# jonas089/toyni

Hardware: AMD Instinct MI355X
Metric: BabyBear NTT throughput (forward+inverse, device-resident) (higher is better)
Workload: dtype u32; 1 GPU; forward+inverse NTT n=2^20 (configs[1]) over a batch of 1024 transforms per GPU (configs[3] repeated-prover batch), in place, inputs resident in HBM; log_n=20, batch_per_gpu=1024, batch_total=1024, passes_per_transform=2, parallelism=batch-sharded x1, no collective

## Files before the change

toyni_amd/csrc/ntt_kernels.hpp:

```cpp
#pragma once
#include "bb_field.hpp"

namespace toyni {

enum PassKind : int { KIND_COL = 0, KIND_ROW_T = 1, KIND_ROW_N = 2 };

struct PassArgs {
    const uint32_t* in;
    uint32_t* out;
    const uint32_t* stage_tw;
    const uint32_t* stage_tw3;
    const uint32_t* tw_lo;
    const uint32_t* tw_hi;
    uint32_t tw_lowbits;
    uint32_t log_S;
    uint32_t scale;
    uint32_t log_n;
    uint32_t log_M1;
    uint32_t log_mid;
    uint64_t rows_total;
    const uint32_t* cs_lo;
    const uint32_t* cs_hi;
    uint32_t cs_lowbits;
    uint32_t cs_mode;
    uint32_t cs_g;
    uint32_t col_base;
    uint32_t in_prefix_log;
    uint32_t nz_rows;
    uint32_t in_split_shift, in_split_extra;
    uint32_t out_split_shift, out_split_extra, out_prefix_log;
    uint32_t row0;
    uint32_t seeds_invariant;
};

#ifndef TOYNI_ABLATE
#define TOYNI_ABLATE 0
#endif

template <bool NT = false>
TOYNI_HD uint32_t ld32(const uint32_t* base, uint32_t byte_off) {
#if TOYNI_ABLATE & 1
    return (uint32_t)(reinterpret_cast<uintptr_t>(base) >> 2) + byte_off;
#elif defined(__HIP_DEVICE_COMPILE__)
    if constexpr (NT) return __builtin_nontemporal_load(reinterpret_cast<const uint32_t*>(reinterpret_cast<const char*>(base) + byte_off));
    else return *reinterpret_cast<const uint32_t*>(reinterpret_cast<const char*>(base) + byte_off);
#else
    return *reinterpret_cast<const uint32_t*>(reinterpret_cast<const char*>(base) + byte_off);
#endif
}
template <bool NT = false>
TOYNI_HD void st32(uint32_t* base, uint32_t byte_off, uint32_t v) {
#if TOYNI_ABLATE & 2
    if (v == 0xFFFFFFFFu)
#endif
#if defined(__HIP_DEVICE_COMPILE__)
// ... 47 lines not shown
    static_assert(LQ_ == 0 || LQ_ == 2, "interleave: none, or the four coordinates of an Ext element");
    static_assert(LQ_ == 0 || KIND == KIND_COL || LC - LQ_ >= (KIND == KIND_ROW_T ? 2 : 3) || LE2 == 0, "interleaved rows: 4 or >= 8 rows per coordinate");
    static constexpr int LM = LE1 + LE2;
    static constexpr int LE1_ = LE1;
    static constexpr int STEPS = LE2 > 0 ? 2 : 1;
    static constexpr int IN_STEP_LOG = LE2, OUT_STEP_LOG = LE2 > 0 ? LE1 : 0;
    static constexpr bool NT = NT_;
    static constexpr uint32_t M = 1u << LM, E1 = 1u << LE1, E2 = 1u << LE2, C = 1u << LC;
    static constexpr uint32_t T = C * E2;
    static constexpr uint32_t G2 = E1 / E2;
    static constexpr bool TWO_STEP = LE2 > 0;

    static constexpr uint32_t PADC = C < 32 ? 32 - C : 0;
    static constexpr uint32_t HI_STRIDE = KIND == KIND_COL ? E2 * C + PADC : E2 + 1;
    static constexpr uint32_t LOW_STRIDE = KIND == KIND_COL ? C : 1;
    static constexpr uint32_t row_pitch() {
        uint32_t base = E1 * (E2 + 1);
        uint32_t want = KIND == KIND_ROW_T ? (C <= 16 ? 2u : 1u) : (LQ_ > 0 ? 1u : (E1 < 32 ? E1 : 0u));
        return base + ((want + 32u - (base & 31u)) & 31u);
    }
    static constexpr uint32_t PITCH = row_pitch();
    static constexpr uint32_t C_STRIDE = KIND == KIND_COL ? 1 : PITCH;
    static constexpr uint32_t LDS_WORDS = !TWO_STEP ? 0 : (KIND == KIND_COL ? E1 * HI_STRIDE : C * PITCH);

    static constexpr uint32_t lds_wg_per_cu() {
        return LDS_WORDS ? (160u * 1024u) / ((LDS_WORDS + (TWO_STEP ? M - E2 : 0u) + ((TWO_STEP && LE1 >= 2 && LC >= 4) ? M - 2u * E2 : 0u)) * 4u) : 8u;
    }
    static constexpr uint32_t min_waves_per_simd() {
        uint32_t w = (lds_wg_per_cu() * (T / 64u ? T / 64u : 1u) + 3u) / 4u;
        return w < 1u ? 1u : (w > 4u ? 4u : w);
    }
    static constexpr uint32_t MIN_WAVES = min_waves_per_simd();

    static TOYNI_HD uint32_t lds_row(uint32_t c) {
        if (LQ_ == 0 || KIND == KIND_COL) return c;
        const uint32_t q = c & (Q - 1u), cc = c >> LQ_;
        if ((C >> LQ_) >= 8u) return (q << 3) + (cc & 7u) + ((cc >> 3) << 5);
        return q * (C >> LQ_) + cc;
    }
    static TOYNI_HD uint32_t lds_word(uint32_t c, uint32_t hi, uint32_t low) { return lds_row(c) * C_STRIDE + hi * HI_STRIDE + low * LOW_STRIDE; }

    struct Tile {
        const uint32_t* in;
        uint32_t* out;
        uint32_t row_shift;
        uint32_t col0;
        uint32_t out0;
        uint32_t valid_c;
        uint32_t bidx;
// ... 100 lines not shown
        return r;
    }
    static TOYNI_HD Twiddle group_twiddle_finish(const PassArgs& a, const TwiddleRaw& r) {
        Twiddle tw{0u, 0u};
        if (KIND == KIND_COL) {
            tw.a0 = mont_mul(r.a_hi, r.a_lo);
            if (a.scale) tw.a0 = mont_mul(tw.a0, a.scale);
            tw.g = mont_mul(r.g_hi, r.g_lo);
        } else if (a.cs_mode == 2u) {
            tw.a0 = mont_mul(r.a_hi, r.a_lo);
            if (KIND == KIND_ROW_N && a.scale) tw.a0 = mont_mul(tw.a0, a.scale);
            tw.g = a.cs_g;
        } else if (SLAB_ && KIND == KIND_ROW_T && a.cs_mode == 4u) {
            tw.a0 = mont_mul(r.a_hi, r.a_lo);
            tw.g = mont_mul(r.g_hi, r.g_lo);
        }
        return tw;
    }
    template <int LSH>
    static TOYNI_HD Twiddle group_twiddle(const PassArgs& a, const Tile& t, uint32_t c, uint32_t khi) {
        return group_twiddle_finish(a, group_twiddle_issue<LSH>(a, t, c, khi));
    }

    template <int LB, int LSH>
    static TOYNI_HD void finish(const PassArgs& a, const Tile& t, uint32_t c, uint32_t khi, Twiddle twd, uint32_t (&x)[1 << LB]) {
        constexpr uint32_t NB = 1u << LB;
        const uint32_t off0 = out_offset(a, c, khi) << 2;
        const uint32_t step = (out_offset(a, 0u, 1u << LSH) - out_offset(a, 0u, 0u)) << 2;
        char* base = reinterpret_cast<char*>(t.out);
#if TOYNI_BUF
        const BufRsrc ws = buf_rsrc(base);
#define TOYNI_STORE(B, V) do { if constexpr (KIND != KIND_ROW_N) stb32<NT_>(ws, off0, (B) * step, (V)); \
                               else st32<NT_>(reinterpret_cast<uint32_t*>(base + (uint64_t)(B) * step), off0, (V)); } while (0)
#else
#define TOYNI_STORE(B, V) st32<NT_>(reinterpret_cast<uint32_t*>(base + (uint64_t)(B) * step), off0, (V))
#endif
        if (KIND == KIND_COL) {
            uint32_t tw = twd.a0;
#pragma unroll
            for (uint32_t b = 0; b < NB; ++b) {
                TOYNI_STORE(b, mont_mul(x[cx_bitrev(b, LB)], tw));
                if (b + 1 < NB) { tw = mont_mul_lazy(tw, twd.g); TOYNI_PIN(tw); }
            }
        } else if (SLAB_ && KIND == KIND_ROW_T) {
            uint32_t tw = twd.a0;
#pragma unroll
            for (uint32_t b = 0; b < NB; ++b) {
                const uint32_t piece = ((b << LSH) >> a.out_split_shift) * (a.out_split_extra << 2);
                uint32_t v = x[cx_bitrev(b, LB)];
                if (a.cs_mode == 4u) {
                    v = mont_mul(v, tw);
                    if (b + 1 < NB) { tw = mont_mul_lazy(tw, twd.g); TOYNI_PIN(tw); }
                }
#if TOYNI_BUF
                stb32<NT_>(ws, off0, b * step + piece, v);
#else
                st32<NT_>(reinterpret_cast<uint32_t*>(base + (uint64_t)b * step + piece), off0, v);
#endif
            }
        } else if (a.cs_mode == 2u) {
// ... 80 lines not shown
                if (q == 0) {
                    x[i + DP] = bb_sub(s0, s1);
                    const uint32_t t = mont_dot_sub(b, e, uni_pow<LE>(uni, QUARTER, false), uni_pow<LE>(uni, QUARTER, true));
                    x[i + D] = bb_add(d0, t);
                    x[i + D + DP] = bb_sub(d0, t);
                } else {
                    const uint32_t d1 = bb_sub(b, e);
                    x[i + DP] = mont_dot_sub(s0, s1, uni_pow<LE>(uni, 2u * q * G, false), uni_pow<LE>(uni, 2u * q * G, true));
                    x[i + D] = mont_dot2(d0, uni_pow<LE>(uni, q * G, false), d1, uni_pow<LE>(uni, q * G + QUARTER, false));
                    x[i + D + DP] = mont_dot2(d0, uni_pow<LE>(uni, 3u * q * G, false), d1, uni_pow<LE>(uni, 3u * q * G + QUARTER, true));
                }
            }
            stages_uniform_r4<LE, S - 2>(x, uni);
        } else if constexpr (S == 0) {
#pragma unroll
            for (uint32_t i = 0; i < (1u << LE); i += 2) {
                const uint32_t u = x[i], v = x[i + 1];
                x[i] = bb_add(u, v);
                x[i + 1] = bb_sub(u, v);
            }
        }
    }

    template <int LE, int SHIFT, int S>
    static TOYNI_HD void stages_thread_r4(uint32_t (&x)[1 << LE], const uint32_t* tw1, const uint32_t* tw3, uint32_t low) {
        TOYNI_PIN(low);
        if constexpr (S >= 1) {
            constexpr int t = S + SHIFT;
            constexpr uint32_t D = 1u << S, DP = 1u << (S - 1), HALF = 1u << (t - 1);
            const uint32_t* t1 = tw1 + ((1u << t) - (1u << SHIFT));
            const uint32_t* t2 = tw1 + (HALF - (1u << SHIFT));
            const uint32_t* t3 = tw3 + ((1u << t) - (2u << SHIFT));
            uint32_t n1 = t1[low], n1p = t1[low + HALF], n2 = t2[low], n3 = t3[low], n3n = t3[HALF + low];
#pragma unroll
            for (uint32_t q = 0; q < DP; ++q) {
                const uint32_t w1 = n1, w1p = n1p, w2 = n2, nw2 = BB_P - n2, w3 = n3, w3n = n3n;
                if (q + 1 < DP) {
                    const uint32_t e1 = low + ((q + 1) << SHIFT);
                    n1 = t1[e1]; n1p = t1[e1 + HALF]; n2 = t2[e1]; n3 = t3[e1]; n3n = t3[HALF + e1];
                }
                TOYNI_SCHED_FENCE();
#pragma unroll
                for (uint32_t hi = 0; hi < (1u << (LE - 1 - S)); ++hi) {
                    const uint32_t i = (hi << (S + 1)) | q;
                    const uint32_t a = x[i], b = x[i + DP], c = x[i + D], e = x[i + D + DP];
                    const uint32_t s0 = bb_add(a, c), s1 = bb_add(b, e), d0 = bb_sub(a, c), d1 = bb_sub(b, e);
                    x[i] = bb_add(s0, s1);
                    x[i + DP] = mont_dot_sub(s0, s1, w2, nw2);
                    x[i + D] = mont_dot2(d0, w1, d1, w1p);
                    x[i + D + DP] = mont_dot2(d0, w3, d1, w3n);
                }
            }
            stages_thread_r4<LE, SHIFT, S - 2>(x, tw1, tw3, low);
        } else if constexpr (S == 0) {
            const uint32_t w = tw1[low], nw = BB_P - w;
#pragma unroll
            for (uint32_t i = 0; i < (1u << LE); i += 2) {
                const uint32_t u = x[i], v = x[i + 1];
                x[i] = bb_add(u, v);
                x[i + 1] = mont_dot_sub(u, v, w, nw);
            }
        }
    }

    template <int LE, int SHIFT, bool R4T = false>
    static TOYNI_HD void stages(uint32_t (&x)[1 << LE], const uint32_t* tw1, uint32_t low, const uint32_t* uni, const uint32_t* tw3 = nullptr) {
#if !defined(TOYNI_NO_RADIX4)
        if constexpr (R4T && SHIFT > 0 && LE >= 2) {
            stages_thread_r4<LE, SHIFT, LE - 1>(x, tw1, tw3, low);
            return;
        }
        if constexpr (SHIFT == 0 && LE >= 2) {
            stages_uniform_r4<LE, LE - 1>(x, uni);
            return;
        }
#endif
#pragma unroll
        for (int s = LE - 1; s >= 0; --s) {
            const int d = 1 << s;
            const int t = s + SHIFT;
            uint32_t w[1 << (LE - 1)], nw[1 << (LE - 1)];
#pragma unroll
// ... 114 lines not shown
            r.lo = a.cs_lo[j0 & ((1u << a.cs_lowbits) - 1u)];
            r.hi = a.cs_hi[j0 >> a.cs_lowbits];
        }
        return r;
    }
    static TOYNI_HD uint32_t in_seed_finish(const PassArgs& a, const InSeedRaw& r) {
        return (KIND != KIND_ROW_T && a.cs_mode == 1u) ? mont_mul(r.hi, r.lo) : 0u;
    }
    template <int LZ = 0>
    static TOYNI_HD void in_scale(const PassArgs& a, const InSeedRaw& r, uint32_t (&x)[E1]) { in_scale_by<LZ>(a, in_seed_finish(a, r), x); }
    template <int LZ = 0>
    static TOYNI_HD void in_scale_by(const PassArgs& a, uint32_t seed, uint32_t (&x)[E1]) {
        constexpr uint32_t NZ = E1 >> (LZ < LE1 ? LZ : LE1);
        if (KIND != KIND_ROW_T && a.cs_mode == 1u) {
            uint32_t tw = seed;
#pragma unroll
            for (uint32_t i = 0; i < NZ; ++i) {
                x[i] = mont_mul(x[i], tw);
                if (i + 1 < NZ) { tw = mont_mul_lazy(tw, a.cs_g); TOYNI_PIN(tw); }
            }
        }
    }

    template <int LZ = 0>
    static TOYNI_HD void step1(const PassArgs& a, const Tile& t, uint32_t tid, uint32_t (&x)[E1], uint32_t* lds, const Uniform& uni,
                               const uint32_t* tw1, const uint32_t* tw3) {
        static_assert(LZ == 0 || TWO_STEP, "zero-padded input needs a two-step pass");
        uint32_t c, lo;
        coords1(tid, c, lo);
        if constexpr (LZ == 0) stages<LE1, LE2, STEP1_R4>(x, tw1, lo, uni.w, tw3);
        else stages_lz<LE1, LE2, LZ, LE1 - 1>(x, tw1, lo, uni.w);
        if (TWO_STEP) {
            const uint32_t base = lds_word(c, 0u, lo);
#pragma unroll
            for (uint32_t i = 0; i < E1; ++i) lds[base + i * HI_STRIDE] = x[i];
        } else {
            if (KIND != KIND_ROW_N || c < t.valid_c) finish<LE1, 0>(a, t, c, 0u, group_twiddle<0>(a, t, c, 0u), x);
        }
    }

    struct SeedsRaw { TwiddleRaw g[G2 ? G2 : 1]; };
    struct Seeds { Twiddle g[G2 ? G2 : 1]; };
    static TOYNI_HD SeedsRaw seeds_issue(const PassArgs& a, const Tile& t, uint32_t tid) {
        SeedsRaw s;
#pragma unroll
        for (uint32_t g = 0; g < G2; ++g) {
            uint32_t c, hi;
            coords2(tid, g, c, hi);
            s.g[g] = group_twiddle_issue<LE1>(a, t, c, bitrev32(hi, LE1));
        }
        return s;
    }
    static TOYNI_HD Seeds seeds_finish(const PassArgs& a, const SeedsRaw& r) {
        Seeds s;
#pragma unroll
        for (uint32_t g = 0; g < G2; ++g) s.g[g] = group_twiddle_finish(a, r.g[g]);
        return s;
    }

    static TOYNI_HD void step2(const PassArgs& a, const Tile& t, uint32_t tid, const uint32_t* lds, const Seeds& seeds, const Uniform& uni) {
#pragma unroll
        for (uint32_t g = 0; g < G2; ++g) {
            uint32_t c, hi;
            coords2(tid, g, c, hi);
            uint32_t x[E2];
            const uint32_t base = lds_word(c, hi, 0u);
#pragma unroll
            for (uint32_t i = 0; i < E2; ++i) x[i] = lds[base + i * LOW_STRIDE];
            stages<LE2, 0>(x, nullptr, 0u, uni.w);
            if (KIND != KIND_ROW_N || c < t.valid_c) finish<LE2, LE1>(a, t, c, bitrev32(hi, LE1), seeds.g[g], x);
        }
    }

    template <int LZ = 0>
    static TOYNI_HD void phase1(const PassArgs& a, uint32_t tile_id, uint32_t tid, uint32_t* lds) {
        const Tile t = tile_of(a, tile_id);
        uint32_t x[E1];
        load_tile<0, E1, LZ>(a, t, tid, x);
        in_scale<LZ>(a, in_seed_issue(a, t, tid), x);
        step1<LZ>(a, t, tid, x, lds, load_uniform(a), tw1_global(a), tw3_global(a));
    }
    static TOYNI_HD void phase2(const PassArgs& a, uint32_t tile_id, uint32_t tid, const uint32_t* lds) {
        const Tile t = tile_of(a, tile_id);
        step2(a, t, tid, lds, seeds_finish(a, seeds_issue(a, t, tid)), load_uniform(a));
    }
};

template <int KIND, int LE1, int LE2, int LE3, int LC, bool NT_ = false, int LQ_ = 0>
struct Pass3 {
    static_assert(KIND == KIND_COL || KIND == KIND_ROW_T, "passes of multi-pass plans");
    static_assert(LQ_ == 0 || (LQ_ == 2 && (LC == 2 || (LC == 4 && LE1 == 5))),
                  "interleaved tiles: one element's four coordinates (latency), or four rows / elements x four coordinates (streaming shapes)");
    static constexpr int LQ = LQ_;
    static_assert(LE1 >= LE2 && LE2 >= LE3 && LE3 >= 1 && LE1 <= 5, "step sizes");
    static constexpr int STEPS = 3;
    static constexpr bool STREAM = LE1 == 5;
    static constexpr int LM = LE1 + LE2 + LE3, LLO = LE2 + LE3, LHM = LE1 + LE2;
    static constexpr int IN_STEP_LOG = LLO, OUT_STEP_LOG = LHM;
    static constexpr bool NT = NT_;
    static constexpr uint32_t M = 1u << LM, E = 1u << LE1, E2 = 1u << LE2, E3 = 1u << LE3, C = 1u << LC;
    static constexpr uint32_t T = C << LLO;
    static constexpr uint32_t G2 = E / E2, G3 = E / E3;
    static_assert(T >= 64 && T <= 1024, "workgroup size");
    using Stg = Pass<KIND_ROW_N, 5, 5, 3>;

    static constexpr uint32_t PADC = C < 32 ? C : 0;
    static constexpr uint32_t PITCH = STREAM ? (M + (M >> LE3)) + ((2u + 32u - ((M + (M >> LE3)) & 31u)) & 31u) : ((M + (M >> LE3)) | 1u);
    static constexpr uint32_t LDS_WORDS = KIND == KIND_COL ? M * C + (M >> LE3) * PADC : C * PITCH;
    static constexpr uint32_t TW_WORDS = M - E3;
    static constexpr bool STEP1_R4 = STREAM;
    static constexpr uint32_t TW1S_WORDS = STREAM ? M - (1u << (LE2 + LE3)) : 0u;
    static constexpr uint32_t TW3S_WORDS = STEP1_R4 ? M - (2u << (LE2 + LE3)) : 0u;
    static constexpr uint32_t MIN_WAVES = 4;
    static constexpr uint32_t STRIDE1 = KIND == KIND_COL ? (C << LLO) + (PADC << LE2) : (1u << LLO) + (1u << LE2);
    static constexpr uint32_t STRIDE2 = KIND == KIND_COL ? (C << LE3) + PADC : E3 + 1u;
    static constexpr uint32_t STRIDE3 = KIND == KIND_COL ? C : 1u;
    static TOYNI_HD uint32_t lds_row(uint32_t c) {
        if (LQ_ == 0 || KIND == KIND_COL || C != 16u) return c;
// ... 742 lines not shown
```

toyni_amd/csrc/ntt_plan.hpp:

```cpp
#pragma once
#include <stdint.h>
#include <type_traits>
#include <vector>

#include "bb_field.hpp"
#include "ntt_kernels.hpp"
#include "ntt_route.hpp"

namespace toyni {

constexpr int MAX_PASSES = 3;
constexpr int MAX_LOG_N = 27;

struct PassPlan {
    int kind;
    int log_m;
    int log_s;
    uint32_t stage_off, stage3_off;
    uint32_t lo_off, hi_off, lowbits;
};

struct NttPlan {
    int log_n = 0;
    int npasses = 0;
// ... 285 lines not shown
    uint32_t log_parts = 0;
    const uint32_t* tw_lo = nullptr;
    const uint32_t* tw_hi = nullptr;
    uint32_t tw_lowbits = 0, row0 = 0;
    bool dry = false;
    bool* unsupported = nullptr;
};

template <class P> struct SlabVariant { using type = P; };
template <int K, int A, int B, int C, bool N, int Q> struct SlabVariant<Pass<K, A, B, C, N, Q, false>> { using type = Pass<K, A, B, C, false, Q, true>; };
template <class P> constexpr bool slab_variant_exists() {
    if constexpr (P::STEPS == 2) return P::PASS_KIND != KIND_ROW_N && P::LQ == 0 && P::C == 32u && P::LM >= 7 && P::LM <= 9 && !P::NT;
    else return false;
}

template <int LQ = 0, class Launch>
inline bool for_each_pass(const LaunchKnobs& k, const NttPlan& plan, const uint32_t* tables, bool inverse, const uint32_t* src,
                          uint32_t* work, uint32_t* dst, uint64_t batch, Launch&& launch, const CosetTables& cs = CosetTables(),
                          int lde_log = 0, bool nt = false, const SlabIo* sio = nullptr) {
    if (plan.log_n == 0 || batch == 0) return true;
    if (sio && (LQ != 0 || lde_log != 0 || cs.lo || plan.npasses < 2 || (batch & (batch - 1)) != 0 || (int)sio->log_parts >= plan.log_n)) return false;
    if (lde_log && (inverse || plan.npasses < 2 || lde_log > plan.pass[0].log_m)) return false;
    const uint64_t total_log = (uint64_t)plan.log_n;
    for (int p = 0; p < plan.npasses; ++p) {
        const PassPlan& pp = plan.pass[p];
        PassArgs a{};
        a.in = p == 0 ? src : work;
        a.out = p == plan.npasses - 1 ? dst : work;
        a.stage_tw = tables + pp.stage_off;
        a.stage_tw3 = tables + pp.stage3_off;
        a.tw_lo = tables + pp.lo_off;
        a.tw_hi = tables + pp.hi_off;
        a.tw_lowbits = pp.lowbits;
        a.log_S = (uint32_t)(pp.log_s + LQ);
        a.in_prefix_log = (uint32_t)(pp.log_s + pp.log_m - (p == 0 ? lde_log : 0) + LQ);
        a.nz_rows = (1u << pp.log_m) >> (p == 0 ? lde_log : 0);
        a.scale = (inverse && p == 0) ? plan.scale_inv : 0u;
        a.log_n = (uint32_t)plan.log_n;
        a.log_M1 = (uint32_t)plan.pass[0].log_m;
        a.log_mid = (uint32_t)(plan.log_n - plan.pass[0].log_m - pp.log_m);
        a.rows_total = batch;
        int log_tiles32 = 0;
        {
            const uint64_t tiles32 = (batch << (total_log - (uint64_t)pp.log_m)) >> 5;
            while ((2ull << log_tiles32) <= tiles32) ++log_tiles32;
        }
        auto body = [&](auto pass, auto lzc) {
            using P = decltype(pass);
            const bool cs_here = cs.lo && (inverse ? p == plan.npasses - 1 : p == 0);
            if (cs_here) {
                a.cs_lo = cs.lo;
                a.cs_hi = cs.hi;
                a.cs_lowbits = cs.lowbits;
                a.cs_mode = inverse ? 2u : 1u;
                uint64_t dj;
                if (!inverse) dj = pp.kind == KIND_COL ? (((uint64_t)1 << P::IN_STEP_LOG) << pp.log_s) : ((uint64_t)1 << P::IN_STEP_LOG);
                else dj = pp.kind == KIND_ROW_T ? ((uint64_t)1 << P::OUT_STEP_LOG) << (plan.log_n - P::LM)
                                                : ((uint64_t)1 << P::OUT_STEP_LOG);
                a.cs_g = to_mont_host(bb_pow_host(cs.s, dj));
            }
            uint64_t nblocks;
            if (pp.kind == KIND_ROW_N) nblocks = (batch + P::C - 1) / P::C;
            else nblocks = (batch << (total_log - P::LM)) / P::C;
            if (sio) {
                const uint32_t log_w = (uint32_t)plan.log_n - sio->log_parts;
                const uint32_t extra = (uint32_t)((batch - 1) << log_w);
                const bool first = p == 0, last = p == plan.npasses - 1;
                bool ok_shape = true;
                const bool special = (!inverse && first) || (inverse && last);
                if (!inverse && first) {
                    ok_shape = slab_variant_exists<P>() && pp.kind == KIND_COL && pp.log_m >= (int)sio->log_parts + P::IN_STEP_LOG;
// ... 6 lines not shown
                    a.out_prefix_log = log_w;
                    a.out_split_shift = (uint32_t)P::LM - sio->log_parts;
                    a.out_split_extra = extra;
                    a.cs_lo = sio->tw_lo;
                    a.cs_hi = sio->tw_hi;
                    a.cs_lowbits = sio->tw_lowbits;
                    a.cs_mode = 4u;
                    a.row0 = sio->row0;
                }
                if (batch == 1) ok_shape = false;
                if (!ok_shape) { if (sio->unsupported) *sio->unsupported = true; return; }
                if (sio->dry || (sio->unsupported && *sio->unsupported)) return;
                if constexpr (slab_variant_exists<P>() && decltype(lzc)::value == 0) {
                    if (special) { launch(typename SlabVariant<P>::type{}, lzc, a, nblocks); return; }
                }
            }
            launch(pass, lzc, a, nblocks);
        };
        bool ok;
        const bool slab_special = sio && ((!inverse && p == 0) || (inverse && p == plan.npasses - 1));
        if (slab_special && log_tiles32 >= k.wide_tiles) log_tiles32 = k.wide_tiles - 1;
        if (p == 0 && lde_log) ok = dispatch_pass_lz<LQ>(k, pp.log_m, log_tiles32, lde_log < 5 ? lde_log : 5, body);
        else ok = dispatch_pass<LQ>(k, pp.kind, pp.log_m, log_tiles32, [&](auto pass) { body(pass, std::integral_constant<int, 0>{}); }, nt && !slab_special);
        if (!ok) return false;
    }
    return true;
}

template <class Launch>
inline bool lds_transform(const NttPlan& plan, const uint32_t* tables, bool inverse, const uint32_t* src, uint32_t* dst, uint64_t batch,
                          Launch&& launch, const CosetTables& cs = CosetTables(), int log_rows = 5) {
    if (!plan.lds_la) return false;
    if (batch == 0) return true;
    LdsArgs g{};
    g.in = src;
    g.out = dst;
    g.stage_a = tables + plan.lds_stage_a_off;
    g.stage_b = tables + plan.lds_stage_b_off;
    g.gtab = tables + plan.lds_gtab_off;
    g.scale = inverse ? plan.scale_inv : 0u;
    g.batch = batch;
    if (cs.lo) {
        g.cs_lo = cs.lo;
        g.cs_hi = cs.hi;
        g.cs_lowbits = cs.lowbits;
        g.cs_mode = inverse ? 2u : 1u;
        g.cs_g = to_mont_host(bb_pow_host(cs.s, inverse ? (32ull << plan.lds_la) : 1024ull));
// ... 73 lines not shown
```

toyni_amd/csrc/ntt_route.hpp:

```cpp
#pragma once
#include <cstdlib>
#include <stdint.h>

namespace toyni {

inline int env_int(const char* name, int dflt) { const char* env = std::getenv(name); return env ? std::atoi(env) : dflt; }
inline uint64_t env_u64(const char* name, uint64_t dflt) { const char* env = std::getenv(name); return env ? (uint64_t)std::strtoull(env, nullptr, 0) : dflt; }

struct LaunchKnobs {
    int p3_tiles = 6;
    int lat_tiles = 7;
    int wide_tiles = 12;
    int s3_tiles = 7;
    bool split_small_first = true;
    int split3[3] = {0, 0, 0};
    int lds_max_log = 13;
    uint64_t lds_min_elems = (uint64_t)1 << 25;
    int lds_rows = 3;
    uint64_t r2048_min_rows = 2048;
    uint64_t r4096_min_rows = 2048;
    uint64_t nt_min_bytes = (uint64_t)512 << 20;

    static LaunchKnobs from_env() {
        LaunchKnobs k;
// ... 14 lines not shown
        if (const char* env = std::getenv("TOYNI_NO_LDS_KERNEL")) if (env[0] == '1') k.lds_max_log = 10;
        k.lds_min_elems = env_u64("TOYNI_LDS_MIN_ELEMS", k.lds_min_elems);
        k.lds_rows = env_int("TOYNI_LDS_ROWS", k.lds_rows);
        k.r2048_min_rows = env_u64("TOYNI_R2048_MIN_ROWS", k.r2048_min_rows);
        k.r4096_min_rows = env_u64("TOYNI_R4096_MIN_ROWS", k.r4096_min_rows);
        k.nt_min_bytes = env_u64("TOYNI_NT_MIN_BYTES", k.nt_min_bytes);
        return k;
    }
};

inline const LaunchKnobs& launch_knobs() {
    static const LaunchKnobs k = LaunchKnobs::from_env();
    return k;
}

constexpr bool seeds_launch_invariant(uint64_t grid, uint64_t ntiles, uint32_t log_S, uint32_t LC) {
    if (grid == 0 || log_S < LC) return false;
    if (grid >= ntiles) return true;
    const uint32_t tiles_log = log_S - LC;
    if (tiles_log == 0) return true;
    if (tiles_log >= 32) return false;
    if ((grid & (((uint64_t)1 << tiles_log) - 1)) != 0) return false;
    return (ntiles & 15) != 0 || (grid & 15) == 0;
}

inline bool has_latency_plan(int log_n) { return log_n == 21 || log_n == 22; }
inline bool has_stream2_plan(int log_n) { return log_n == 21; }

template <class Plan> inline bool row2048_enabled(const Plan& plan, uint64_t batch, const LaunchKnobs& k) {
    if (batch < 1) return false;
    return (plan.log_n == 11 && batch >= k.r2048_min_rows) || (plan.log_n == 12 && batch >= k.r4096_min_rows);
}
template <class Plan> inline bool lds_kernel_enabled(const Plan& plan, uint64_t batch, const LaunchKnobs& k) {
    return plan.lds_la != 0 && plan.log_n <= k.lds_max_log && (batch << plan.log_n) >= k.lds_min_elems;
}

template <class Plan> inline bool use_two_pass_plan(const Plan& plan, const Plan* plan_lat, uint64_t batch, int lq, int lde_log, const LaunchKnobs& k) {
    if (!plan_lat) return false;
    if (lde_log != 0 && lde_log > plan_lat->pass[0].log_m) return false;
    if (lq != 0) return (has_stream2_plan(plan.log_n) || (lde_log != 0 && has_latency_plan(plan.log_n))) && k.s3_tiles <= 7;
    const bool lat_small = k.p3_tiles >= 0 && k.lat_tiles >= 0 &&
                           ((batch << (plan.log_n - plan_lat->pass[0].log_m)) >> 5) <= (1ull << k.lat_tiles);
    const bool lat_stream = k.s3_tiles < 99 && (has_stream2_plan(plan.log_n) || (lde_log != 0 && has_latency_plan(plan.log_n)));
    return lat_small || lat_stream;
}

// ... 46 lines not shown
```

toyni_amd/csrc/toyni_hip.hip:

```cpp
#ifndef TOYNI_KERNEL_TEXT_ONLY
#include <hip/hip_runtime.h>

#include <cstdio>
#include <cstdlib>
#include <atomic>
#include <chrono>
#include <cstring>
#include <map>
#include <mutex>
#include <string>
#include <thread>
#include <vector>

#ifdef TOYNI_TOOLS
#include "toyni_hip_tools.h"
#endif
#endif
#include "toyni_hip.h"
#include "ntt_plan.hpp"
#include "merkle_kernels.hpp"
#include "prover_kernels.hpp"

using namespace toyni;

// ... 13 lines not shown
}
#undef hipLaunchKernelGGL
#define hipLaunchKernelGGL(kernel, grid, block, shmem, stream, ...)                                      \
    do {                                                                                                 \
        static std::atomic<bool> _toyni_site_seen{false};                                                \
        if (!_toyni_site_seen.load(std::memory_order_acquire)) {                                         \
            if (launch_registry::note(reinterpret_cast<const void*>(kernel)))                            \
                _toyni_site_seen.store(true, std::memory_order_release);                                 \
        }                                                                                                \
        kernel<<<(grid), (block), (shmem), (stream)>>>(__VA_ARGS__);                                     \
    } while (0)

#define HIPCHK(expr)                                 \
    do {                                               \
        hipError_t _e = (expr);                        \
        if (_e != hipSuccess) return (int)_e;          \
    } while (0)
#endif

template <class P> struct PassKindOf;
template <int K, int A, int B, int C, bool N, int Q, bool S> struct PassKindOf<Pass<K, A, B, C, N, Q, S>> { static constexpr int value = K; };
template <class P> constexpr int kind_of() { return PassKindOf<P>::value; }

template <class P, int PF, int LZ = 0>
__global__ void __launch_bounds__(P::T, P::MIN_WAVES) ntt_pass_kernel(const PassArgs a, const uint32_t ntiles) {
    __shared__ uint32_t lds[(P::LDS_WORDS + P::TW1_WORDS + P::TW3_WORDS) ? (P::LDS_WORDS + P::TW1_WORDS + P::TW3_WORDS) : 1];
    const uint32_t tid = threadIdx.x;
    if constexpr (!P::TWO_STEP) {
        static_assert(LZ == 0, "single-step passes take whole inputs");
        for (uint32_t v = blockIdx.x; v < ntiles; v += gridDim.x) P::phase1(a, P::tile_order(v, ntiles), tid, lds);
    } else {
        constexpr uint32_t NPF = PF < 0 ? 0u : ((uint32_t)PF > P::E1 ? P::E1 : (uint32_t)PF);
        uint32_t v = blockIdx.x;
        if (v >= ntiles) return;
        uint32_t* lds_tw1 = lds + P::LDS_WORDS;
        uint32_t* lds_tw3 = lds_tw1 + P::TW1_WORDS;
        uint32_t x[P::E1];
        typename P::Tile t = P::tile_of(a, P::tile_order(v, ntiles));
        P::template load_tile<0, NPF, LZ>(a, t, tid, x);
        typename P::SeedsRaw raw = P::seeds_issue(a, t, tid);
        typename P::InSeedRaw inraw = P::in_seed_issue(a, t, tid);
        const typename P::Uniform uni = P::load_uniform(a);
        for (uint32_t j = tid; j < P::TW1_WORDS; j += P::T) lds_tw1[j] = P::tw1_global(a)[j];
        for (uint32_t j = tid; j < P::TW3_WORDS; j += P::T) lds_tw3[j] = P::tw3_global(a)[j];
        TOYNI_WAIT_VMEM0();
        __syncthreads();
        const bool hoist = kind_of<P>() == KIND_COL && !P::SLAB && a.seeds_invariant != 0u;
        typename P::Seeds seeds = P::seeds_finish(a, raw);
        uint32_t inseed = P::in_seed_finish(a, inraw);
        while (true) {
            static_assert(P::G2 * P::E2 == P::E1 && P::E1 <= 63, "stores per tile per thread");
            if constexpr (kind_of<P>() != KIND_ROW_N) TOYNI_WAIT_VMEM_ALLOW(P::E1);
            else TOYNI_WAIT_VMEM0();
            P::template load_tile<NPF, P::E1, LZ>(a, t, tid, x);
            if (!hoist) inseed = P::in_seed_finish(a, inraw);
            P::template in_scale_by<LZ>(a, inseed, x);
            P::template step1<LZ>(a, t, tid, x, lds, uni, lds_tw1, lds_tw3);
            if (!hoist) seeds = P::seeds_finish(a, raw);
#pragma unroll
            for (uint32_t g = 0; g < P::G2; ++g) { TOYNI_PIN(seeds.g[g].a0); TOYNI_PIN(seeds.g[g].g); }
            TOYNI_SCHED_FENCE();
            const uint32_t vn = v + gridDim.x;
            const bool more = vn < ntiles;
            typename P::Tile tn = t;
            if (more) {
                tn = P::tile_of(a, P::tile_order(vn, ntiles));
                P::template load_tile<0, NPF, LZ>(a, tn, tid, x);
                if (!hoist) {
                    raw = P::seeds_issue(a, tn, tid);
                    inraw = P::in_seed_issue(a, tn, tid);
                }
            }
            TOYNI_SCHED_FENCE();
            TOYNI_LDS_BARRIER();
            TOYNI_SCHED_FENCE();
            P::step2(a, t, tid, lds, seeds, uni);
            if (!more) break;
            TOYNI_SCHED_FENCE();
            TOYNI_BARRIER();
            TOYNI_SCHED_FENCE();
            t = tn;
            v = vn;
        }
    }
}

template <class P, int LZ = 0>
__global__ void __launch_bounds__(P::T, P::MIN_WAVES) ntt_pass3_kernel(const PassArgs a, const uint32_t ntiles) {
    __shared__ uint32_t lds[P::LDS_WORDS + P::TW_WORDS];
    const uint32_t tid = threadIdx.x;
    uint32_t v = blockIdx.x;
    if (v >= ntiles) return;
    uint32_t* lds_tw = lds + P::LDS_WORDS;
    constexpr uint32_t TW_REGS = (P::TW_WORDS + P::T - 1) / P::T;
    uint32_t tw_regs[TW_REGS];
#pragma unroll
    for (uint32_t k = 0; k < TW_REGS; ++k) {
        const uint32_t j = tid + k * P::T;
        tw_regs[k] = j < P::TW_WORDS ? P::tw_global(a)[j] : 0u;
    }
    const typename P::Uniform uni = P::load_uniform(a);
    bool first = true;
    while (true) {
        const typename P::Tile t = P::tile_of(a, P::tile_order(v, ntiles));
        uint32_t x[P::E];
// ... 1485 lines not shown
    }
    (void)hipGetLastError();
    (void)hipThreadExchangeStreamCaptureMode(&cmode);
    for (size_t i = 0; i < c->retired.size(); ++i)
        if (!c->retired[i].ptr) drop_retired_event(c, i);
    size_t keep = 0;
    for (auto& r : c->retired)
        if (r.ptr) c->retired[keep++] = r;
    c->retired.resize(keep);
}

int grid_for(size_t items, int block = 256) {
    size_t g = (items + block - 1) / block;
    const size_t cap = 256 * 8;
    return (int)(g < 1 ? 1 : (g > cap ? cap : g));
}

template <class P> constexpr int ext_prefetch() { return (kind_of<P>() == KIND_ROW_N && P::LM == 10) ? 0 : 32; }

template <class P> constexpr bool hoists_seeds() {
    if constexpr (P::STEPS == 2) return kind_of<P>() == KIND_COL && !P::SLAB;
    else return false;
}

template <class P> constexpr uint32_t log_tile_width() {
    uint32_t l = 0;
    while ((1u << l) < P::C) ++l;
    return l;
}

template <class P, int LZ = 0>
void launch_pass(unsigned grid, hipStream_t s, const PassArgs& args, uint32_t ntiles) {
    PassArgs a = args;
    if constexpr (hoists_seeds<P>()) a.seeds_invariant = seeds_launch_invariant(grid, ntiles, a.log_S, log_tile_width<P>()) ? 1u : 0u;
    if constexpr (P::STEPS == 3) {
        if constexpr (P::STREAM) hipLaunchKernelGGL((ntt_pass3s_kernel<P, LZ>), dim3(grid), dim3(P::T), 0, s, a, ntiles);
        else hipLaunchKernelGGL((ntt_pass3_kernel<P, LZ>), dim3(grid), dim3(P::T), 0, s, a, ntiles);
    } else if constexpr (LZ > 0) {
        hipLaunchKernelGGL((ntt_pass_kernel<P, 32, LZ>), dim3(grid), dim3(P::T), 0, s, a, ntiles);
    } else if constexpr (P::LQ > 0) {
        hipLaunchKernelGGL((ntt_pass_kernel<P, ext_prefetch<P>()>), dim3(grid), dim3(P::T), 0, s, a, ntiles);
    } else {
        hipLaunchKernelGGL((ntt_pass_kernel<P, 32>), dim3(grid), dim3(P::T), 0, s, a, ntiles);
    }
}

template <class P, int LZ = 0>
unsigned persistent_grid(toyni_ntt_ctx* c, uint64_t ntiles) {
    static const int per_cu = [] {
        int occ = 0;
        hipError_t qe;
        if constexpr (P::STEPS == 3) {
            if constexpr (P::STREAM) qe = hipOccupancyMaxActiveBlocksPerMultiprocessor(&occ, ntt_pass3s_kernel<P, LZ>, (int)P::T, 0);
            else qe = hipOccupancyMaxActiveBlocksPerMultiprocessor(&occ, ntt_pass3_kernel<P, 0>, (int)P::T, 0);
        } else if constexpr (P::LQ > 0) qe = hipOccupancyMaxActiveBlocksPerMultiprocessor(&occ, ntt_pass_kernel<P, ext_prefetch<P>()>, (int)P::T, 0);
        else qe = hipOccupancyMaxActiveBlocksPerMultiprocessor(&occ, ntt_pass_kernel<P, 32>, (int)P::T, 0);
        if (qe != hipSuccess || occ < 1) occ = 1;
        if (const int v = env_int("TOYNI_WG_PER_CU", 0); v > 0) occ = v;
        return occ;
    }();
    uint64_t g = (uint64_t)c->num_cus * (uint64_t)per_cu;
    if (g > ntiles) g = ntiles;
    if (g >= 16) g &= ~(uint64_t)15;
    return (unsigned)(g < 1 ? 1 : g);
// ... 2061 lines not shown
```

Baseline: 306.7 billion elements/s.

## Fold inter-pass twiddle multiply into the closing row pass for 2^20 NTT

For the two-pass 1024x1024 plan, the column pass now stores plain outputs without the per-element twiddle multiply. The twiddles are instead folded into the first radix-4 stage of the row pass, which uses a per-tile LDS table of G factors. The final radix-2 stage then applies the A factor together with the inverse scale. This removes a separate multiply chain in the column pass. In exchange it adds an LDS table, per-tile twiddle loads, and mont_dot2 butterflies in the row pass, which may reduce occupancy.

```diff
diff --git a/toyni_amd/csrc/ntt_kernels.hpp b/toyni_amd/csrc/ntt_kernels.hpp
--- a/toyni_amd/csrc/ntt_kernels.hpp
+++ b/toyni_amd/csrc/ntt_kernels.hpp
@@ -31,6 +31,7 @@
     uint32_t out_split_shift, out_split_extra, out_prefix_log;
     uint32_t row0;
     uint32_t seeds_invariant;
+    uint32_t fold_tw;
 };
 
 #ifndef TOYNI_ABLATE
@@ -124,9 +125,15 @@
     static constexpr uint32_t PITCH = row_pitch();
     static constexpr uint32_t C_STRIDE = KIND == KIND_COL ? 1 : PITCH;
     static constexpr uint32_t LDS_WORDS = !TWO_STEP ? 0 : (KIND == KIND_COL ? E1 * HI_STRIDE : C * PITCH);
+#if defined(TOYNI_NO_RADIX4) || defined(TOYNI_NO_RADIX4_THREAD)
+    static constexpr bool FOLD_SHAPE = false;
+#else
+    static constexpr bool FOLD_SHAPE = (KIND == KIND_COL || KIND == KIND_ROW_T) && LE1 == 5 && LE2 == 5 && LC == 5 && LQ_ == 0 && !SLAB_;
+#endif
+    static constexpr uint32_t G_WORDS = (FOLD_SHAPE && KIND == KIND_ROW_T) ? C * E1 : 0;
 
     static constexpr uint32_t lds_wg_per_cu() {
-        return LDS_WORDS ? (160u * 1024u) / ((LDS_WORDS + (TWO_STEP ? M - E2 : 0u) + ((TWO_STEP && LE1 >= 2 && LC >= 4) ? M - 2u * E2 : 0u)) * 4u) : 8u;
+        return LDS_WORDS ? (160u * 1024u) / ((LDS_WORDS + (TWO_STEP ? M - E2 : 0u) + ((TWO_STEP && LE1 >= 2 && LC >= 4) ? M - 2u * E2 : 0u) + G_WORDS) * 4u) : 8u;
     }
     static constexpr uint32_t min_waves_per_simd() {
         uint32_t w = (lds_wg_per_cu() * (T / 64u ? T / 64u : 1u) + 3u) / 4u;
@@ -273,7 +280,7 @@
         return group_twiddle_finish(a, group_twiddle_issue<LSH>(a, t, c, khi));
     }
 
-    template <int LB, int LSH>
+    template <int LB, int LSH, bool PLAIN = false>
     static TOYNI_HD void finish(const PassArgs& a, const Tile& t, uint32_t c, uint32_t khi, Twiddle twd, uint32_t (&x)[1 << LB]) {
         constexpr uint32_t NB = 1u << LB;
         const uint32_t off0 = out_offset(a, c, khi) << 2;
@@ -286,7 +293,11 @@
 #else
 #define TOYNI_STORE(B, V) st32<NT_>(reinterpret_cast<uint32_t*>(base + (uint64_t)(B) * step), off0, (V))
 #endif
-        if (KIND == KIND_COL) {
+        if constexpr (PLAIN) {
+            static_assert(KIND == KIND_COL, "plain stores: the column pass of a folded plan");
+#pragma unroll
+            for (uint32_t b = 0; b < NB; ++b) TOYNI_STORE(b, x[cx_bitrev(b, LB)]);
+        } else if (KIND == KIND_COL) {
             uint32_t tw = twd.a0;
 #pragma unroll
             for (uint32_t b = 0; b < NB; ++b) {
@@ -413,8 +424,20 @@
         }
     }
 
-    template <int LE, int SHIFT, int S>
-    static TOYNI_HD void stages_thread_r4(uint32_t (&x)[1 << LE], const uint32_t* tw1, const uint32_t* tw3, uint32_t low) {
+    struct GQuad { uint32_t a, b, c, e; };
+    static TOYNI_HD GQuad load_gquad(const uint32_t* grow, uint32_t q) {
+#if defined(__HIP_DEVICE_COMPILE__)
+        typedef uint32_t u32x4_a16 __attribute__((ext_vector_type(4)));
+        const u32x4_a16 v = *reinterpret_cast<const u32x4_a16*>(grow + 4u * q);
+        return GQuad{v.x, v.y, v.z, v.w};
+#else
+        return GQuad{grow[4u * q], grow[4u * q + 1u], grow[4u * q + 2u], grow[4u * q + 3u]};
+#endif
+    }
+    template <int LE, int SHIFT, int S, bool FOLD = false>
+    static TOYNI_HD void stages_thread_r4(uint32_t (&x)[1 << LE], const uint32_t* tw1, const uint32_t* tw3, uint32_t low, const uint32_t* grow = nullptr,
+                                          uint32_t fa = 0u) {
+        static_assert(!FOLD || (LE >= 3 && (LE & 1)), "the fold: G on the first group, A on the single last stage");
         TOYNI_PIN(low);
         if constexpr (S >= 1) {
             constexpr int t = S + SHIFT;
@@ -422,33 +445,45 @@
             const uint32_t* t1 = tw1 + ((1u << t) - (1u << SHIFT));
             const uint32_t* t2 = tw1 + (HALF - (1u << SHIFT));
             const uint32_t* t3 = tw3 + ((1u << t) - (2u << SHIFT));
+            constexpr bool GIN = FOLD && S == LE - 1;
             uint32_t n1 = t1[low], n1p = t1[low + HALF], n2 = t2[low], n3 = t3[low], n3n = t3[HALF + low];
+            GQuad ng{0u, 0u, 0u, 0u};
+            if constexpr (GIN) ng = load_gquad(grow, 0u);
 #pragma unroll
             for (uint32_t q = 0; q < DP; ++q) {
                 const uint32_t w1 = n1, w1p = n1p, w2 = n2, nw2 = BB_P - n2, w3 = n3, w3n = n3n;
+                const GQuad g = ng;
                 if (q + 1 < DP) {
                     const uint32_t e1 = low + ((q + 1) << SHIFT);
                     n1 = t1[e1]; n1p = t1[e1 + HALF]; n2 = t2[e1]; n3 = t3[e1]; n3n = t3[HALF + e1];
+                    if constexpr (GIN) ng = load_gquad(grow, q + 1u);
                 }
                 TOYNI_SCHED_FENCE();
 #pragma unroll
                 for (uint32_t hi = 0; hi < (1u << (LE - 1 - S)); ++hi) {
                     const uint32_t i = (hi << (S + 1)) | q;
                     const uint32_t a = x[i], b = x[i + DP], c = x[i + D], e = x[i + D + DP];
-                    const uint32_t s0 = bb_add(a, c), s1 = bb_add(b, e), d0 = bb_sub(a, c), d1 = bb_sub(b, e);
+                    uint32_t s0, s1, d0, d1;
+                    if constexpr (GIN) {
+                        const uint32_t ngc = BB_P - g.c, nge = BB_P - g.e;
+                        s0 = mont_dot2(a, g.a, c, g.c); s1 = mont_dot2(b, g.b, e, g.e);
+                        d0 = mont_dot2(a, g.a, c, ngc); d1 = mont_dot2(b, g.b, e, nge);
+                    } else {
+                        s0 = bb_add(a, c); s1 = bb_add(b, e); d0 = bb_sub(a, c); d1 = bb_sub(b, e);
+                    }
                     x[i] = bb_add(s0, s1);
                     x[i + DP] = mont_dot_sub(s0, s1, w2, nw2);
                     x[i + D] = mont_dot2(d0, w1, d1, w1p);
                     x[i + D + DP] = mont_dot2(d0, w3, d1, w3n);
                 }
             }
-            stages_thread_r4<LE, SHIFT, S - 2>(x, tw1, tw3, low);
+            stages_thread_r4<LE, SHIFT, S - 2, FOLD>(x, tw1, tw3, low, grow, fa);
         } else if constexpr (S == 0) {
-            const uint32_t w = tw1[low], nw = BB_P - w;
+            const uint32_t w = FOLD ? mont_mul(tw1[low], fa) : tw1[low], nw = BB_P - w;
 #pragma unroll
             for (uint32_t i = 0; i < (1u << LE); i += 2) {
                 const uint32_t u = x[i], v = x[i + 1];
-                x[i] = bb_add(u, v);
+                x[i] = FOLD ? mont_mul(u + v, fa) : bb_add(u, v);
                 x[i + 1] = mont_dot_sub(u, v, w, nw);
             }
         }
@@ -609,13 +644,32 @@
         }
     }
 
-    template <int LZ = 0>
-    static TOYNI_HD void step1(const PassArgs& a, const Tile& t, uint32_t tid, uint32_t (&x)[E1], uint32_t* lds, const Uniform& uni,
-                               const uint32_t* tw1, const uint32_t* tw3) {
-        static_assert(LZ == 0 || TWO_STEP, "zero-padded input needs a two-step pass");
+    struct InTwiddleRaw { uint32_t a_lo, a_hi, g_lo, g_hi; };
+    static TOYNI_HD InTwiddleRaw in_twiddle_issue(const PassArgs& a, const Tile& t, uint32_t tid) {
         uint32_t c, lo;
         coords1(tid, c, lo);
-        if constexpr (LZ == 0) stages<LE1, LE2, STEP1_R4>(x, tw1, lo, uni.w, tw3);
+        const uint32_t mask = (1u << a.tw_lowbits) - 1u;
+        const uint32_t ea = (t.out0 + c) * lo, eg = ea << LE2;
+        return InTwiddleRaw{a.tw_lo[ea & mask], a.tw_hi[ea >> a.tw_lowbits], a.tw_lo[eg & mask], a.tw_hi[eg >> a.tw_lowbits]};
+    }
+    static constexpr uint32_t g_word(uint32_t i) { return ((i & (E1 / 4u - 1u)) << 2) | (i >> (LE1 - 2)); }
+    static TOYNI_HD uint32_t in_twiddle_finish(const PassArgs& a, const InTwiddleRaw& r, uint32_t* gtab, uint32_t tid) {
+        uint32_t c, lo;
+        coords1(tid, c, lo);
+        gtab[c * E1 + g_word(lo)] = mont_mul(r.g_hi, r.g_lo);
+        const uint32_t fa = mont_mul(r.a_hi, r.a_lo);
+        return a.scale ? mont_mul(fa, a.scale) : fa;
+    }
+
+    template <int LZ = 0, bool FOLD = false>
+    static TOYNI_HD void step1(const PassArgs& a, const Tile& t, uint32_t tid, uint32_t (&x)[E1], uint32_t* lds, const Uniform& uni,
+                               const uint32_t* tw1, const uint32_t* tw3, const uint32_t* gtab = nullptr, uint32_t fa = 0u) {
+        static_assert(LZ == 0 || TWO_STEP, "zero-padded input needs a two-step pass");
+        static_assert(!FOLD || (FOLD_SHAPE && KIND == KIND_ROW_T && LZ == 0), "input twiddle: the closing shape of a folded plan");
+        uint32_t c, lo;
+        coords1(tid, c, lo);
+        if constexpr (FOLD) stages_thread_r4<LE1, LE2, LE1 - 1, true>(x, tw1, tw3, lo, gtab + c * E1, fa);
+        else if constexpr (LZ == 0) stages<LE1, LE2, STEP1_R4>(x, tw1, lo, uni.w, tw3);
         else stages_lz<LE1, LE2, LZ, LE1 - 1>(x, tw1, lo, uni.w);
         if (TWO_STEP) {
             const uint32_t base = lds_word(c, 0u, lo);
@@ -645,6 +699,7 @@
         return s;
     }
 
+    template <bool PLAIN = false>
     static TOYNI_HD void step2(const PassArgs& a, const Tile& t, uint32_t tid, const uint32_t* lds, const Seeds& seeds, const Uniform& uni) {
 #pragma unroll
         for (uint32_t g = 0; g < G2; ++g) {
@@ -655,7 +710,7 @@
 #pragma unroll
             for (uint32_t i = 0; i < E2; ++i) x[i] = lds[base + i * LOW_STRIDE];
             stages<LE2, 0>(x, nullptr, 0u, uni.w);
-            if (KIND != KIND_ROW_N || c < t.valid_c) finish<LE2, LE1>(a, t, c, bitrev32(hi, LE1), seeds.g[g], x);
+            if (KIND != KIND_ROW_N || c < t.valid_c) finish<LE2, LE1, PLAIN>(a, t, c, bitrev32(hi, LE1), seeds.g[g], x);
         }
     }
 
@@ -665,10 +720,27 @@
         uint32_t x[E1];
         load_tile<0, E1, LZ>(a, t, tid, x);
         in_scale<LZ>(a, in_seed_issue(a, t, tid), x);
+        if constexpr (FOLD_SHAPE && KIND == KIND_ROW_T && LZ == 0) {
+            if (a.fold_tw) {
+                uint32_t c, lo, fa = 0u;
+                coords1(tid, c, lo);
+                uint32_t gtab[C * E1];
+                for (uint32_t i = 0; i < E1; ++i) {
+                    const uint32_t other = (tid - lo) + i;
+                    const uint32_t f = in_twiddle_finish(a, in_twiddle_issue(a, t, other), gtab, other);
+                    if (i == lo) fa = f;
+                }
+                step1<0, true>(a, t, tid, x, lds, load_uniform(a), tw1_global(a), tw3_global(a), gtab, fa);
+                return;
+            }
+        }
         step1<LZ>(a, t, tid, x, lds, load_uniform(a), tw1_global(a), tw3_global(a));
     }
     static TOYNI_HD void phase2(const PassArgs& a, uint32_t tile_id, uint32_t tid, const uint32_t* lds) {
         const Tile t = tile_of(a, tile_id);
+        if constexpr (FOLD_SHAPE && KIND == KIND_COL) {
+            if (a.fold_tw) { step2<true>(a, t, tid, lds, Seeds{}, load_uniform(a)); return; }
+        }
         step2(a, t, tid, lds, seeds_finish(a, seeds_issue(a, t, tid)), load_uniform(a));
     }
 };
@@ -681,6 +753,7 @@
     static constexpr int LQ = LQ_;
     static_assert(LE1 >= LE2 && LE2 >= LE3 && LE3 >= 1 && LE1 <= 5, "step sizes");
     static constexpr int STEPS = 3;
+    static constexpr bool FOLD_SHAPE = false;
     static constexpr bool STREAM = LE1 == 5;
     static constexpr int LM = LE1 + LE2 + LE3, LLO = LE2 + LE3, LHM = LE1 + LE2;
     static constexpr int IN_STEP_LOG = LLO, OUT_STEP_LOG = LHM;
diff --git a/toyni_amd/csrc/ntt_plan.hpp b/toyni_amd/csrc/ntt_plan.hpp
--- a/toyni_amd/csrc/ntt_plan.hpp
+++ b/toyni_amd/csrc/ntt_plan.hpp
@@ -331,6 +331,8 @@
     if (sio && (LQ != 0 || lde_log != 0 || cs.lo || plan.npasses < 2 || (batch & (batch - 1)) != 0 || (int)sio->log_parts >= plan.log_n)) return false;
     if (lde_log && (inverse || plan.npasses < 2 || lde_log > plan.pass[0].log_m)) return false;
     const uint64_t total_log = (uint64_t)plan.log_n;
+    const bool fold = fold_twiddle_into_closing(plan, batch, LQ, lde_log, sio != nullptr, k);
+    bool fold_shape_ok = true;
     for (int p = 0; p < plan.npasses; ++p) {
         const PassPlan& pp = plan.pass[p];
         PassArgs a{};
@@ -349,6 +351,13 @@
         a.log_M1 = (uint32_t)plan.pass[0].log_m;
         a.log_mid = (uint32_t)(plan.log_n - plan.pass[0].log_m - pp.log_m);
         a.rows_total = batch;
+        if (fold) {
+            a.fold_tw = 1u;
+            a.tw_lo = tables + plan.pass[0].lo_off;
+            a.tw_hi = tables + plan.pass[0].hi_off;
+            a.tw_lowbits = plan.pass[0].lowbits;
+            a.scale = (inverse && p == plan.npasses - 1) ? plan.scale_inv : 0u;
+        }
         int log_tiles32 = 0;
         {
             const uint64_t tiles32 = (batch << (total_log - (uint64_t)pp.log_m)) >> 5;
@@ -356,6 +365,7 @@
         }
         auto body = [&](auto pass, auto lzc) {
             using P = decltype(pass);
+            if (fold && !P::FOLD_SHAPE) { fold_shape_ok = false; return; }
             const bool cs_here = cs.lo && (inverse ? p == plan.npasses - 1 : p == 0);
             if (cs_here) {
                 a.cs_lo = cs.lo;
@@ -408,7 +418,7 @@
         if (slab_special && log_tiles32 >= k.wide_tiles) log_tiles32 = k.wide_tiles - 1;
         if (p == 0 && lde_log) ok = dispatch_pass_lz<LQ>(k, pp.log_m, log_tiles32, lde_log < 5 ? lde_log : 5, body);
         else ok = dispatch_pass<LQ>(k, pp.kind, pp.log_m, log_tiles32, [&](auto pass) { body(pass, std::integral_constant<int, 0>{}); }, nt && !slab_special);
-        if (!ok) return false;
+        if (!ok || !fold_shape_ok) return false;
     }
     return true;
 }
diff --git a/toyni_amd/csrc/ntt_route.hpp b/toyni_amd/csrc/ntt_route.hpp
--- a/toyni_amd/csrc/ntt_route.hpp
+++ b/toyni_amd/csrc/ntt_route.hpp
@@ -60,6 +60,25 @@
     if (tiles_log >= 32) return false;
     if ((grid & (((uint64_t)1 << tiles_log) - 1)) != 0) return false;
     return (ntiles & 15) != 0 || (grid & 15) == 0;
+}
+
+constexpr bool row_tile_launch_invariant(uint64_t grid, uint64_t ntiles, uint32_t log_M1, uint32_t log_mid, uint32_t LC) {
+    return log_mid == 0 && seeds_launch_invariant(grid, ntiles, log_M1, LC);
+}
+
+template <class Plan> inline bool fold_twiddle_into_closing(const Plan& plan, uint64_t batch, int lq, int lde_log, bool pieces, const LaunchKnobs& k) {
+#if defined(TOYNI_NO_RADIX4) || defined(TOYNI_NO_RADIX4_THREAD)
+    (void)plan; (void)batch; (void)lq; (void)lde_log; (void)pieces; (void)k;
+    return false;
+#else
+    if (plan.npasses != 2 || plan.log_n != 20 || plan.pass[0].log_m != 10 || plan.pass[1].log_m != 10) return false;
+    if (lq != 0 || lde_log != 0 || pieces) return false;
+    const uint64_t tiles32 = (batch << 10) >> 5;
+    if (tiles32 < ((uint64_t)1 << 9)) return false;
+    int log_tiles32 = 9;
+    while (((uint64_t)2 << log_tiles32) <= tiles32) ++log_tiles32;
+    return !(k.p3_tiles >= 0 && log_tiles32 <= k.p3_tiles);
+#endif
 }
 
 inline bool has_latency_plan(int log_n) { return log_n == 21 || log_n == 22; }
diff --git a/toyni_amd/csrc/toyni_hip.hip b/toyni_amd/csrc/toyni_hip.hip
--- a/toyni_amd/csrc/toyni_hip.hip
+++ b/toyni_amd/csrc/toyni_hip.hip
@@ -59,10 +59,13 @@
 template <int K, int A, int B, int C, bool N, int Q, bool S> struct PassKindOf<Pass<K, A, B, C, N, Q, S>> { static constexpr int value = K; };
 template <class P> constexpr int kind_of() { return PassKindOf<P>::value; }
 
-template <class P, int PF, int LZ = 0>
+template <class P, int PF, int LZ = 0, bool FOLD = false>
 __global__ void __launch_bounds__(P::T, P::MIN_WAVES) ntt_pass_kernel(const PassArgs a, const uint32_t ntiles) {
-    __shared__ uint32_t lds[(P::LDS_WORDS + P::TW1_WORDS + P::TW3_WORDS) ? (P::LDS_WORDS + P::TW1_WORDS + P::TW3_WORDS) : 1];
+    constexpr uint32_t G_WORDS = FOLD ? P::G_WORDS : 0u;
+    __shared__ __align__(16) uint32_t lds[(P::LDS_WORDS + P::TW1_WORDS + P::TW3_WORDS + G_WORDS) ? (P::LDS_WORDS + P::TW1_WORDS + P::TW3_WORDS + G_WORDS) : 1];
     const uint32_t tid = threadIdx.x;
+    constexpr bool FOLD_COL = FOLD && kind_of<P>() == KIND_COL, FOLD_ROW = FOLD && kind_of<P>() == KIND_ROW_T;
+    static_assert(!FOLD || (LZ == 0 && P::FOLD_SHAPE), "the fold: whole inputs, the 32-wide 1024-point base-field shapes");
     if constexpr (!P::TWO_STEP) {
         static_assert(LZ == 0, "single-step passes take whole inputs");
         for (uint32_t v = blockIdx.x; v < ntiles; v += gridDim.x) P::phase1(a, P::tile_order(v, ntiles), tid, lds);
@@ -72,17 +75,24 @@
         if (v >= ntiles) return;
         uint32_t* lds_tw1 = lds + P::LDS_WORDS;
         uint32_t* lds_tw3 = lds_tw1 + P::TW1_WORDS;
+        uint32_t* lds_g = lds_tw3 + P::TW3_WORDS;
+        static_assert(!FOLD_ROW || ((P::LDS_WORDS + P::TW1_WORDS + P::TW3_WORDS) & 3u) == 0, "16-byte reads of the input-twiddle table");
+        const bool fold_per_tile = FOLD_ROW && a.seeds_invariant == 0u;
+        typename P::InTwiddleRaw graw{0u, 0u, 0u, 0u};
+        uint32_t fa = 0u, fa_next = 0u;
         uint32_t x[P::E1];
         typename P::Tile t = P::tile_of(a, P::tile_order(v, ntiles));
         P::template load_tile<0, NPF, LZ>(a, t, tid, x);
         typename P::SeedsRaw raw = P::seeds_issue(a, t, tid);
         typename P::InSeedRaw inraw = P::in_seed_issue(a, t, tid);
+        if constexpr (FOLD_ROW) graw = P::in_twiddle_issue(a, t, tid);
         const typename P::Uniform uni = P::load_uniform(a);
         for (uint32_t j = tid; j < P::TW1_WORDS; j += P::T) lds_tw1[j] = P::tw1_global(a)[j];
         for (uint32_t j = tid; j < P::TW3_WORDS; j += P::T) lds_tw3[j] = P::tw3_global(a)[j];
         TOYNI_WAIT_VMEM0();
+        if constexpr (FOLD_ROW) fa = P::in_twiddle_finish(a, graw, lds_g, tid);
         __syncthreads();
-        const bool hoist = kind_of<P>() == KIND_COL && !P::SLAB && a.seeds_invariant != 0u;
+        const bool hoist = FOLD_COL || (kind_of<P>() == KIND_COL && !P::SLAB && a.seeds_invariant != 0u);
         typename P::Seeds seeds = P::seeds_finish(a, raw);
         uint32_t inseed = P::in_seed_finish(a, inraw);
         while (true) {
@@ -92,7 +102,11 @@
             P::template load_tile<NPF, P::E1, LZ>(a, t, tid, x);
             if (!hoist) inseed = P::in_seed_finish(a, inraw);
             P::template in_scale_by<LZ>(a, inseed, x);
-            P::template step1<LZ>(a, t, tid, x, lds, uni, lds_tw1, lds_tw3);
+            if constexpr (FOLD_ROW) {
+                P::template step1<0, true>(a, t, tid, x, lds, uni, lds_tw1, lds_tw3, lds_g, fa);
+            } else {
+                P::template step1<LZ>(a, t, tid, x, lds, uni, lds_tw1, lds_tw3);
+            }
             if (!hoist) seeds = P::seeds_finish(a, raw);
 #pragma unroll
             for (uint32_t g = 0; g < P::G2; ++g) { TOYNI_PIN(seeds.g[g].a0); TOYNI_PIN(seeds.g[g].g); }
@@ -107,17 +121,20 @@
                     raw = P::seeds_issue(a, tn, tid);
                     inraw = P::in_seed_issue(a, tn, tid);
                 }
+                if constexpr (FOLD_ROW) { if (fold_per_tile) graw = P::in_twiddle_issue(a, tn, tid); }
             }
             TOYNI_SCHED_FENCE();
             TOYNI_LDS_BARRIER();
             TOYNI_SCHED_FENCE();
-            P::step2(a, t, tid, lds, seeds, uni);
+            if constexpr (FOLD_ROW) { if (fold_per_tile && more) fa_next = P::in_twiddle_finish(a, graw, lds_g, tid); }
+            P::template step2<FOLD_COL>(a, t, tid, lds, seeds, uni);
             if (!more) break;
             TOYNI_SCHED_FENCE();
             TOYNI_BARRIER();
             TOYNI_SCHED_FENCE();
             t = tn;
             v = vn;
+            if constexpr (FOLD_ROW) { if (fold_per_tile) fa = fa_next; }
         }
     }
 }
@@ -1649,6 +1666,10 @@
     if constexpr (P::STEPS == 2) return kind_of<P>() == KIND_COL && !P::SLAB;
     else return false;
 }
+template <class P> constexpr bool folds_rows() {
+    if constexpr (P::STEPS == 2) return kind_of<P>() == KIND_ROW_T && P::FOLD_SHAPE;
+    else return false;
+}
 
 template <class P> constexpr uint32_t log_tile_width() {
     uint32_t l = 0;
@@ -1660,6 +1681,7 @@
 void launch_pass(unsigned grid, hipStream_t s, const PassArgs& args, uint32_t ntiles) {
     PassArgs a = args;
     if constexpr (hoists_seeds<P>()) a.seeds_invariant = seeds_launch_invariant(grid, ntiles, a.log_S, log_tile_width<P>()) ? 1u : 0u;
+    if constexpr (folds_rows<P>()) a.seeds_invariant = (a.fold_tw && row_tile_launch_invariant(grid, ntiles, a.log_M1, a.log_mid, log_tile_width<P>())) ? 1u : 0u;
     if constexpr (P::STEPS == 3) {
         if constexpr (P::STREAM) hipLaunchKernelGGL((ntt_pass3s_kernel<P, LZ>), dim3(grid), dim3(P::T), 0, s, a, ntiles);
         else hipLaunchKernelGGL((ntt_pass3_kernel<P, LZ>), dim3(grid), dim3(P::T), 0, s, a, ntiles);
@@ -1667,6 +1689,9 @@
         hipLaunchKernelGGL((ntt_pass_kernel<P, 32, LZ>), dim3(grid), dim3(P::T), 0, s, a, ntiles);
     } else if constexpr (P::LQ > 0) {
         hipLaunchKernelGGL((ntt_pass_kernel<P, ext_prefetch<P>()>), dim3(grid), dim3(P::T), 0, s, a, ntiles);
+    } else if constexpr (P::FOLD_SHAPE) {
+        if (a.fold_tw) hipLaunchKernelGGL((ntt_pass_kernel<P, 32, 0, true>), dim3(grid), dim3(P::T), 0, s, a, ntiles);
+        else hipLaunchKernelGGL((ntt_pass_kernel<P, 32>), dim3(grid), dim3(P::T), 0, s, a, ntiles);
     } else {
         hipLaunchKernelGGL((ntt_pass_kernel<P, 32>), dim3(grid), dim3(P::T), 0, s, a, ntiles);
     }
```

New measurement: 308.7 billion elements/s, median of 6. About the same (+0.7%).
